# nico-bohlinger/RL-X

Hardware: AMD Instinct MI355X
Metric: env-steps/sec (whole node) PPO 4096 envs at 1/2/4/8 MI355X (higher is better)
Workload: dtype f32

## Files before the change

rl-x_amd/csrc/common.h:

```cpp
#pragma once
#include <hip/hip_runtime.h>
#include <hip/hip_ext.h>
#include <stdint.h>
#include <cstring>
#include <cmath>
#include <string>
#include <vector>
#include <functional>
#include "../../include/rlx_hip.h"

namespace rlx {

void set_error(const std::string& msg);

#define RLX_HIP_TRY(expr)                                                                      \
  do {                                                                                         \
    hipError_t e_ = (expr);                                                                    \
    if (e_ != hipSuccess) {                                                                    \
      ::rlx::set_error(std::string(#expr) + " failed: " + hipGetErrorString(e_) + " (" __FILE__ \
                       ":" + std::to_string(__LINE__) + ")");                                  \
      return RLX_EHIP;                                                                         \
    }                                                                                          \
  } while (0)

// ... 68 lines not shown
  bool pipeline_updates = true;
  bool pf_valid = false;
  uint32_t pf_key_in[2] = {0, 0}, pf_key_out[2] = {0, 0};
  int pf_E = 0, pf_scheme = 0;
  int64_t pf_B = 0;
  hipEvent_t pf_done = nullptr;
  hipEvent_t ev_perm_free = nullptr;
  bool perm_free_recorded = false;
  bool two_streams = true;
  const uint32_t* l1_xmax = nullptr;
  const uint32_t* xmax_slot[2] = {nullptr, nullptr};
  int lf_idle_cus = 0;
  bool dw_recompute = false;
  float* l12_stats = nullptr;
  bool l12_ran = false;
  bool dw_merge = true;
  void* dbg_stamps = nullptr;
  bool fwd2h = true;
  int gather_group_rows = 524288;
  bool gather_records = true;
  bool l12_fused = true;
  int ppo_tail = -1;
  int tail32_waves = 8;
  int ln_row_once = 1;
  int ppo_twin = -1;
  bool fused_recurrent_act = true;
  int num_cus = 256;
  void* defer = nullptr;
  bool prof_on = false;
  int prof_sample = 1;
// ... 376 lines not shown
```

rl-x_amd/csrc/core.hip:

```cpp
#include "common.h"
#include <algorithm>
#include <cstdio>
#include <cstdlib>
#include <utility>

namespace rlx {

static thread_local std::string g_last_error;

void set_error(const std::string& msg) { g_last_error = msg; }

void* scratch(rlx_ctx* ctx, ScratchSlot s, size_t bytes) {
  Scratch& sl = ctx->slots[ctx->bank][s];
  if (sl.bytes >= bytes && sl.ptr) return sl.ptr;
  if (sl.ptr) {
    if (hipDeviceSynchronize() != hipSuccess) { set_error("hipDeviceSynchronize failed in scratch()"); return nullptr; }
    (void)hipFree(sl.ptr);
    sl.ptr = nullptr;
    sl.bytes = 0;
  }
  size_t want = ((bytes > (size_t(1) << 20) ? bytes + bytes / 8 : bytes) + 255) & ~size_t(255);
  void* p = nullptr;
  hipError_t e = hipMalloc(&p, want);
  if (e != hipSuccess) {
// ... 201 lines not shown
  if (std::string(name) == "fwd2h") { ctx->fwd2h = value != 0; return RLX_OK; }
  if (std::string(name) == "l12_fused") { ctx->l12_fused = value != 0; return RLX_OK; }
  if (std::string(name) == "gather_group_rows") { ctx->gather_group_rows = value; return RLX_OK; }
  if (std::string(name) == "gather_records") { ctx->gather_records = value != 0; return RLX_OK; }
  if (std::string(name) == "ppo_tail") { ctx->ppo_tail = value < 0 ? -1 : (value > 2 ? 2 : value); return RLX_OK; }
  if (std::string(name) == "tail32_waves") {
    RLX_REQUIRE(value == 4 || value == 8, RLX_EINVAL, "rlx_dbg_set_option: tail32_waves is 4 or 8");
    ctx->tail32_waves = value;
    return RLX_OK;
  }
  if (std::string(name) == "ln_row_once") {
    RLX_REQUIRE(value == 0 || value == 1, RLX_EINVAL, "rlx_dbg_set_option: ln_row_once is 0 or 1");
    ctx->ln_row_once = value;
    return RLX_OK;
  }
  if (std::string(name) == "bx_force_mi") { ctx->bx_force_mi = value; return RLX_OK; }
  if (std::string(name) == "adam_emit") { ctx->adam_emit = value != 0; return RLX_OK; }
  if (std::string(name) == "bx_debug") { ctx->bx_debug = value; return RLX_OK; }
  if (std::string(name) == "bx_gscale_log2") { ctx->bx_gscale = ldexpf(1.f, value < 0 ? 0 : (value > 40 ? 40 : value)); return RLX_OK; }
  if (std::string(name) == "gemm_bx") { ctx->gemm_bx = value != 0; return RLX_OK; }
  if (std::string(name) == "prof_sample") { ctx->prof_sample = value < 1 ? 1 : value; return RLX_OK; }
  if (std::string(name) == "espo_chunk") { ctx->espo_chunk = value < 1 ? 1 : value; return RLX_OK; }
  if (std::string(name) == "fused_recurrent_act") { ctx->fused_recurrent_act = value != 0; return RLX_OK; }
  RLX_REQUIRE(false, RLX_EINVAL, "rlx_dbg_set_option: unknown option");
}

int rlx_dbg_get_counter(rlx_ctx* ctx, const char* name, int64_t* out) {
  RLX_REQUIRE(ctx && name && out, RLX_EINVAL, "rlx_dbg_get_counter: NULL");
  int bank = 0, slot = 0;
  if (sscanf(name, "scratch_ptr:%d:%d", &bank, &slot) == 2 && bank >= 0 && bank < 3 && slot >= 0 && slot < rlx::SL_COUNT) {
// ... 78 lines not shown
```

rl-x_amd/csrc/l1fused.hip:

```cpp
#include <type_traits>

#include "mlp.h"
#include "gemm_bx.h"

namespace rlx {

#ifndef RLX_LF_PFX
#define RLX_LF_PFX 2
#endif
#ifndef RLX_LF_DWSCALE
#define RLX_LF_DWSCALE 1
#endif
#ifndef RLX_LF_ABL
#define RLX_LF_ABL 0
#endif
#ifndef RLX_LF_STAMPS
#define RLX_LF_STAMPS 0
#endif
constexpr int LF_ROWS = 32;
constexpr int LF_THREADS = 256;
constexpr int LF_XS = 33;
constexpr int LFP_N2 = 256;

typedef float lf_v4 __attribute__((ext_vector_type(4)));
// ... 22 lines not shown
  const float* dZ2;
  const float* W2t;
  const float* W1;
  const float* b1;
  const float* g;
  const float* be;
  float* partials;
  int64_t M;
  int O, H1, N2, act, ln;
  const void* W2x;
  int NTx;
  float gs, gso;
  const void* W1x;
  const uint32_t* xmax;
  unsigned long long* stamps;
};

__device__ __forceinline__ int lf_bx_off(int r, int ks, int N2) { return r * 2 * N2 + ((ks ^ (r & 15)) << 4); }
__device__ __forceinline__ void lf_bx_stage4(char* __restrict__ img, int r, int c4, lf_v4 v, int N2, float sc) {
  uint32_t a0, a1, b0, b1;
  bx_split2(v[0] * sc, v[1] * sc, a0, a1);
  bx_split2(v[2] * sc, v[3] * sc, b0, b1);
  char* d = img + lf_bx_off(r, c4 >> 3, N2) + ((c4 & 4) << 1);
  const int plane = LF_ROWS * 2 * N2;
  *reinterpret_cast<u32x2*>(d) = u32x2{a0, b0};
  *reinterpret_cast<u32x2*>(d + plane) = u32x2{a1, b1};
}

constexpr int LF_XPLANE = LF_ROWS * X_ROWB;
constexpr int LF_XIMG = 2 * X_NP * LF_XPLANE;
__device__ __forceinline__ void lf_x_stage(char* __restrict__ img, int r, int k, float v, float xs) {
  uint32_t p0, p1;
  bx_split2(v * xs, 0.f, p0, p1);
  const int pos = (r & ~12) | ((r & 4) << 1) | ((r & 8) >> 1);
  char* da = img + bx_off(r, k >> 3) + (k & 7) * 2;
  char* dt = img + X_NP * LF_XPLANE + bx_off(k, pos >> 3) + (pos & 7) * 2;
  *reinterpret_cast<uint16_t*>(da) = (uint16_t)p0;
  *reinterpret_cast<uint16_t*>(da + LF_XPLANE) = (uint16_t)p1;
  *reinterpret_cast<uint16_t*>(dt) = (uint16_t)p0;
  *reinterpret_cast<uint16_t*>(dt + LF_XPLANE) = (uint16_t)p1;
}

template <int NT, int NW, int ACT, bool LN, bool BX, bool TWIN = false, bool ROW1 = false>
__global__ __launch_bounds__(64 * NW, NW / 4) void k_dx_l1bwd(L1FusedArgs a, L1FusedArgs a2) {
  if (TWIN && blockIdx.y) a = a2;
  static_assert(!ROW1 || LN, "ROW1 is a form of the LayerNorm statistics");
  constexpr int H1 = 32 * NT * NW;
  constexpr int NTHREADS = 64 * NW;
  extern __shared__ __attribute__((aligned(16))) float smem[];
  const int OP = (a.O + 1) & ~1;
  float* W1s = smem;
  const bool dbuf = a.N2 == LFP_N2;
  const int nbuf = dbuf ? 2 : 1;
  float* As0 = W1s + (BX ? 0 : OP * H1);
  const int a_img = BX ? X_NP * LF_ROWS * a.N2 / 2 : LF_ROWS * (a.N2 + 4);
  float* Xs0 = As0 + nbuf * a_img;
  const int x_img = BX ? LF_XIMG / 4 : LF_ROWS * LF_XS;
  float* red = Xs0 + nbuf * x_img;
  const int t = threadIdx.x, lane = t & 63, w = t >> 6, li = lane & 31, lh = lane >> 5;
  const bool lb0 = (lane & 1) != 0, lb1 = (lane & 2) != 0;
  const int O = a.O, N2 = a.N2;
// ... 21 lines not shown
  }
  const float invH = 1.0f / (float)H1;
  float dw_scale = (RLX_LF_DWSCALE && LN) ? 0.f : a.gs;
  const int AS = N2 + 4;
  const int nq = N2 >> 3;
  constexpr int PF = 4;
  const lf_v4* __restrict__ Wf = reinterpret_cast<const lf_v4*>(a.W2t);
  const u32x4* __restrict__ Wx = reinterpret_cast<const u32x4*>(a.W2x) + (int64_t)(w * NT) * X_NP * 64 + lane;
  const int wx_step = a.NTx * X_NP * 64;
  const u32x4* __restrict__ W1x = reinterpret_cast<const u32x4*>(a.W1x) + (int64_t)(w * NT) * X_NP * 64 + lane;

  const int64_t ntiles = (a.M + LF_ROWS - 1) / LF_ROWS;
  constexpr int SA_N = LF_ROWS * (LFP_N2 / 4) / NTHREADS, SX_N = LF_ROWS * 32 / NTHREADS;
  lf_v4 sa[SA_N];
  float sx[SX_N];
  auto stage_load = [&](int64_t tl) {
    const int64_t rr = tl * LF_ROWS;
#pragma unroll
    for (int c = 0; c < SA_N; ++c) {
      const int i = t + c * NTHREADS, r = i / (LFP_N2 / 4), c4 = (i % (LFP_N2 / 4)) * 4;
      sa[c] = (rr + r < a.M) ? *reinterpret_cast<const lf_v4*>(a.dZ2 + (rr + r) * LFP_N2 + c4) : lf_v4{0.f, 0.f, 0.f, 0.f};
    }
#pragma unroll
    for (int c = 0; c < SX_N; ++c) {
      const int i = t + c * NTHREADS, r = i >> 5, k = i & 31;
      sx[c] = (k < O && rr + r < a.M) ? a.X[(rr + r) * O + k] : 0.f;
    }
  };
  auto stage_store = [&](int b) {
    float* Ad = As0 + b * a_img;
    float* Xd = Xs0 + b * x_img;
#pragma unroll
    for (int c = 0; c < SA_N; ++c) {
      const int i = t + c * NTHREADS, r = i / (LFP_N2 / 4), c4 = (i % (LFP_N2 / 4)) * 4;
      if (BX) lf_bx_stage4(reinterpret_cast<char*>(Ad), r, c4, sa[c], LFP_N2, a.gs);
      else *reinterpret_cast<lf_v4*>(Ad + r * (LFP_N2 + 4) + c4) = sa[c];
    }
#pragma unroll
    for (int c = 0; c < SX_N; ++c) {
      const int i = t + c * NTHREADS;
      if (BX) lf_x_stage(reinterpret_cast<char*>(Xd), i >> 5, i & 31, sx[c], xs);
      else Xd[(i >> 5) * LF_XS + (i & 31)] = sx[c];
    }
  };
  if (dbuf && (int64_t)blockIdx.x < ntiles) {
    stage_load(blockIdx.x);
    stage_store(0);
  }
  int buf = 0;
#if RLX_LF_STAMPS
  int sti = 0;
#define LF_STAMP() if (a.stamps && t == 0 && blockIdx.x == 0 && blockIdx.y == 0 && sti < 18) a.stamps[sti++] = clock64();
#define LF_WALL(I) if (a.stamps && t == 0 && blockIdx.x == 0 && blockIdx.y == 0) a.stamps[I] = wall_clock64();
#define LF_WALL_END() if (sti == 17) { LF_WALL(19) }
#else
#define LF_STAMP()
#define LF_WALL(I)
#define LF_WALL_END()
// ... 30 lines not shown
    if (dbuf) {
      if (has_next) stage_load(tile + gridDim.x);
    } else {
      for (int i = t; i < LF_ROWS * 32; i += NTHREADS) {
        const int r = i >> 5, k = i & 31;
        const float xv = (k < O && r0 + r < a.M) ? a.X[(r0 + r) * O + k] : 0.f;
        if (BX) lf_x_stage(reinterpret_cast<char*>(Xs), r, k, xv, xs);
        else Xs[r * LF_XS + k] = xv;
      }
      for (int i = t; i < LF_ROWS * (N2 >> 2); i += NTHREADS) {
        const int r = i / (N2 >> 2), c4 = (i - r * (N2 >> 2)) * 4;
        const lf_v4 v = (r0 + r < a.M) ? *reinterpret_cast<const lf_v4*>(a.dZ2 + (r0 + r) * N2 + c4) : lf_v4{0.f, 0.f, 0.f, 0.f};
        if (BX) lf_bx_stage4(reinterpret_cast<char*>(As), r, c4, v, N2, a.gs);
        else *reinterpret_cast<lf_v4*>(As + r * AS + c4) = v;
      }
      __syncthreads();
    }
    LF_STAMP()
    const float* a0 = As + li * AS + 4 * lh;
    if (RLX_LF_ABL & 1) {
    } else if (BX) {
      const char* img = reinterpret_cast<const char*>(As);
      const int plane = LF_ROWS * 2 * N2, nb16 = N2 >> 4;
      for (int q = 0; q < nb16; q += PFX) {
#pragma unroll
        for (int u = 0; u < PFX; ++u) {
          u32x4 av[X_NP];
          const char* ab = img + lf_bx_off(li, 2 * (q + u) + lh, N2);
#pragma unroll
          for (int p = 0; p < X_NP; ++p) av[p] = *reinterpret_cast<const u32x4*>(ab + p * plane);
// ... 74 lines not shown
      for (int j = 0; j < NT; ++j)
#pragma unroll
        for (int r = 0; r < 16; ++r) z[j][r] = bias[j];
      const float* x0 = Xs + li * LF_XS + lh;
      const float* w0 = W1s + lh * H1 + w * 32 * NT + li;
      for (int kk = 0; kk < ((RLX_LF_ABL & 8) ? 0 : OP); kk += 2) {
        const float av = x0[kk];
#pragma unroll
        for (int j = 0; j < NT; ++j)
          z[j] = __builtin_amdgcn_mfma_f32_32x32x2f32(av, w0[kk * H1 + 32 * j], z[j], 0, 0, 0);
      }
    }
    LF_STAMP()
    constexpr bool red_on = ln;
    float* redA = red;
    float* redB = red + 2 * NW * 32;
    float* totA = redB + 2 * NW * 32 + w * 64;
    float* totB = redB + 2 * NW * 32 + NW * 64 + w * 64;
    if (red_on) {
#pragma unroll
      for (int g = 0; g < 4; ++g) {
        float sv[4], ssv[4];
#pragma unroll
        for (int e = 0; e < 4; ++e) {
          const int r = 4 * g + e;
          float s = 0.f, ss = 0.f;
#pragma unroll
          for (int j = 0; j < NT; ++j) { s += z[j][r]; ss += z[j][r] * z[j][r]; }
          sv[e] = s;
          ssv[e] = ss;
        }
        const float st = half_sum4(sv[0], sv[1], sv[2], sv[3], lb0, lb1);
        const float sst = half_sum4(ssv[0], ssv[1], ssv[2], ssv[3], lb0, lb1);
        if (li < 4) {
          redA[(0 * NW + w) * 32 + 8 * g + 4 * lh + li] = st;
          redA[(1 * NW + w) * 32 + 8 * g + 4 * lh + li] = sst;
        }
      }
      __syncthreads();
      float rs_row = 0.f;
      {
        float v = 0.f;
#pragma unroll
        for (int q = 0; q < NW; ++q) v += redA[((lane >> 5) * NW + q) * 32 + (lane & 31)];
        totA[lane] = ROW1 ? ln_row_stats(v, lane, invH, rs_row) : v;
      }
      if (BX && RLX_LF_DWSCALE && dw_scale == 0.f) {
        float rs;
        if (ROW1) {
          rs = rs_row;
        } else {
          const float mean = totA[lane & 31] * invH;
          rs = rsqrtf(fmaxf(0.f, totA[32 + (lane & 31)] * invH - mean * mean) + 1e-6f);
        }
        if (r0 + (lane & 31) >= a.M) rs = 0.f;
        rs = fmaxf(rs, dpp_f(rs, 0));
        rs = fmaxf(rs, dpp_f(rs, 1));
        rs = fmaxf(rs, dpp_f(rs, 2));
        rs = fmaxf(rs, dpp_f(rs, 3));
        const unsigned u = (unsigned)__float_as_int(rs);
        const auto r16 = __builtin_amdgcn_permlane16_swap(u, u, false, false);
        rs = fmaxf(__int_as_float((int)r16[0]), __int_as_float((int)r16[1]));
        dw_scale = a.gs * x_pow2_inv(__int_as_float(__builtin_amdgcn_readfirstlane(__float_as_int(rs))));
      }
// ... 128 lines not shown
    {
      const unsigned u0 = (unsigned)__float_as_int(v0), u1 = (unsigned)__float_as_int(v1), u2 = (unsigned)__float_as_int(v2);
      const auto s0 = __builtin_amdgcn_permlane32_swap(u0, u0, false, false);
      const auto s1 = __builtin_amdgcn_permlane32_swap(u1, u1, false, false);
      const auto s2 = __builtin_amdgcn_permlane32_swap(u2, u2, false, false);
      v0 = __int_as_float((int)s0[0]) + __int_as_float((int)s0[1]);
      v1 = __int_as_float((int)s1[0]) + __int_as_float((int)s1[1]);
      v2 = __int_as_float((int)s2[0]) + __int_as_float((int)s2[1]);
    }
    if (lh == 0) {
      out[(int64_t)O * H1 + col] = v0;
      out[(int64_t)(O + 1) * H1 + col] = v1;
      out[(int64_t)(O + 2) * H1 + col] = v2;
    }
  }
}

template <int NT, int NW, int ACT, bool LN, int KS>
__global__ __launch_bounds__(64 * NW, 2) void k_l1fwd_mfma(const float* __restrict__ X, const float* __restrict__ W1,
                                                           const float* __restrict__ b1, const float* __restrict__ g,
                                                           const float* __restrict__ be, float* __restrict__ Hout,
                                                           int64_t M, int O, const int32_t* __restrict__ m_dev,
                                                           int64_t pdelta, float* __restrict__ Hout1) {
  if (blockIdx.y) { W1 += pdelta; b1 += pdelta; g += pdelta; be += pdelta; Hout = Hout1; }
  if (m_dev && (int64_t)*m_dev < M) M = *m_dev;
  constexpr int H1 = 32 * NT * NW;
  constexpr int NTHREADS = 64 * NW;
  extern __shared__ __attribute__((aligned(16))) float smem[];
  const int OP = (O + 1) & ~1;
  float* Xs = smem;
// ... 365 lines not shown
  }
#undef L12_STAMP
#undef L12_WALL
}

bool l12fwd_supported(const rlx_mlp_desc& d) {
  return l1fwd_mfma_supported(d) && d.n_hidden >= 2 && (d.hidden[1] == 256 || d.hidden[1] == 512);
}

int launch_l12fwd(rlx_ctx* ctx, const rlx_mlp_desc& d, const MlpLayout& L, const float* params, const float* x, float* h1, float* h2,
                  const void* w1x, const void* w2x, int64_t M, hipStream_t st, const L12Twin* tw, float* stats) {
  const bool row1 = ctx->ln_row_once != 0;
  const LayerOff &o0 = L.layer[0], &o1 = L.layer[1];
  L12Args a;
  a.X = x; a.W1x = w1x; a.b1 = params + o0.b; a.g = params + o0.g; a.be = params + o0.be; a.W2x = w2x; a.b2 = params + o1.b;
  a.H1 = stats ? nullptr : h1; a.H2 = h2; a.stats = stats; a.xmax = ctx->l1_xmax; a.M = M; a.O = o0.in;
  a.stamps = (unsigned long long*)ctx->dbg_stamps;
  L12Args a2 = a;
  if (tw) {
    a2.W1x = tw->w1x; a2.b1 = tw->params + o0.b; a2.g = tw->params + o0.g; a2.be = tw->params + o0.be; a2.W2x = tw->w2x;
    a2.b2 = tw->params + o1.b; a2.H1 = stats ? nullptr : tw->h1; a2.H2 = tw->h2; a2.stats = tw->stats;
  }
  const int N2 = o1.out;
  const double nets = tw ? 2.0 : 1.0;
  ProfScope prof(ctx, PK_L12FWD, nets * 2.0 * (double)M * L12_H1 * (N2 + o0.in), st,
                 nets * 4.0 * ((double)M * (o0.in + (stats ? 2 : L12_H1) + N2) + (double)L12_H1 * (N2 + o0.in)), M, N2, L12_H1, 1);
  const int64_t nt = (M + LF_ROWS - 1) / LF_ROWS;
  const int per = tw ? ctx->num_cus : 2 * ctx->num_cus;
  const int grid = (int)(nt < per ? nt : per);
  const size_t lds = (size_t)X_NP * LF_ROWS * L12_AROW + 2 * X_NP * LF_XPLANE + (2 * 8 * 32 + 8 * 64) * sizeof(float);
#define RLX_L12_ATTR(...)                                                                                          \
  RLX_HIP_TRY(hipFuncSetAttribute(reinterpret_cast<const void*>(k_l12fwd<__VA_ARGS__>), hipFuncAttributeMaxDynamicSharedMemorySize, 160 * 1024));
#define RLX_L12_LAUNCH_ROW(NT2V, ROWV)                                                                             \
  {                                                                                                                \
    static AttrOnce attr_set;                                                                                        \
    if (!attr_set.done()) {                                                                                               \
      RLX_L12_ATTR(RLX_ACT_ELU, NT2V, false, false, ROWV)                                                          \
      RLX_L12_ATTR(RLX_ACT_ELU, NT2V, true, false, ROWV)                                                           \
      RLX_L12_ATTR(RLX_ACT_ELU, NT2V, false, true, ROWV)                                                           \
      attr_set.mark();                                                                                               \
    }                                                                                                              \
// ... 92 lines not shown
                       H1, N2);
    RLX_LAUNCH_CHECK();
  }
  L1FusedArgs a;
  a.X = x; a.dZ2 = dZ2; a.W2t = W2t; a.W1 = params + o0.W; a.b1 = params + o0.b;
  a.g = o0.g >= 0 ? params + o0.g : nullptr;
  a.be = o0.be >= 0 ? params + o0.be : nullptr;
  a.partials = slabs; a.M = M; a.O = O; a.H1 = H1; a.N2 = N2; a.act = d.act; a.ln = d.ln_first ? 1 : 0;
  a.W2x = w2x;
  a.W1x = w1x;
  a.NTx = 4 * div_up(H1, G_BN);
  a.gs = ctx->bx_gscale;
  a.gso = X_WINV / a.gs;
  a.xmax = ctx->l1_xmax;
  a.stamps = RLX_LF_STAMPS ? (unsigned long long*)ctx->dbg_stamps : nullptr;
  L1FusedArgs a2 = a;
  if (tw) {
    a2.dZ2 = tw->dZ2; a2.W1 = tw->params + o0.W; a2.b1 = tw->params + o0.b;
    a2.g = o0.g >= 0 ? tw->params + o0.g : nullptr;
    a2.be = o0.be >= 0 ? tw->params + o0.be : nullptr;
    a2.partials = tw->arena; a2.W2x = tw->w2x; a2.W1x = tw->w1x;
  }
  const int OP = (O + 1) & ~1;
  const size_t a_img = bxk ? (size_t)X_NP * LF_ROWS * N2 / 2 : (size_t)LF_ROWS * (N2 + 4);
  const size_t lds = bxk ? ((N2 == LFP_N2 ? 2 : 1) * (a_img + LF_XIMG / 4) + 2048) * sizeof(float)
                         : ((size_t)OP * H1 + (N2 == LFP_N2 ? 2 : 1) * (a_img + LF_ROWS * LF_XS) + 2048) * sizeof(float);
  RLX_REQUIRE(lds <= 160 * 1024, RLX_EUNSUP, "l1fused: tile image exceeds the LDS");
  {
    const double ntw = tw ? 2.0 : 1.0;
    ProfScope prof(ctx, PK_DX_L1BWD, ntw * 2.0 * (double)M * H1 * (N2 + O), st,
                   ntw * 4.0 * ((double)M * N2 + (double)H1 * N2 + (double)M * O + 2.0 * O * H1), M, H1, N2, bxk ? 1 : 0);
#define RLX_LF_ATTR(KERNEL)                                                                                    \
  {                                                                                                            \
    static AttrOnce attr_set;                                                                                    \
    if (!attr_set.done()) {                                                                                           \
      RLX_HIP_TRY(hipFuncSetAttribute(reinterpret_cast<const void*>(KERNEL), hipFuncAttributeMaxDynamicSharedMemorySize, \
                                      160 * 1024));                                                            \
      attr_set.mark();                                                                                           \
    }                                                                                                          \
  }
#define RLX_LF_LAUNCH(NTV, NWV, ACTV, LNV)                                                                      \
  {                                                                                                            \
    RLX_LF_ATTR((k_dx_l1bwd<NTV, NWV, ACTV, LNV, false>))                                                      \
    RLX_LF_ATTR((k_dx_l1bwd<NTV, NWV, ACTV, LNV, true>))                                                       \
    RLX_LF_ATTR((k_dx_l1bwd<NTV, NWV, ACTV, LNV, true, true>))                                                 \
    if (tw) { RLX_PLAUNCH((k_dx_l1bwd<NTV, NWV, ACTV, LNV, true, true>), dim3(grid, 2), dim3(64 * NWV), lds, st, a, a2); } \
    else if (bxk) { RLX_PLAUNCH((k_dx_l1bwd<NTV, NWV, ACTV, LNV, true>), dim3(grid), dim3(64 * NWV), lds, st, a, a2); } \
    else { RLX_PLAUNCH((k_dx_l1bwd<NTV, NWV, ACTV, LNV, false>), dim3(grid), dim3(64 * NWV), lds, st, a, a2); }    \
  }
#define RLX_LF_LAUNCH_ROW1(NTV, NWV, ACTV)                                                                      \
  {                                                                                                            \
    RLX_LF_ATTR((k_dx_l1bwd<NTV, NWV, ACTV, true, true, false, true>))                                         \
    RLX_LF_ATTR((k_dx_l1bwd<NTV, NWV, ACTV, true, true, true, true>))                                          \
    if (tw) { RLX_PLAUNCH((k_dx_l1bwd<NTV, NWV, ACTV, true, true, true, true>), dim3(grid, 2), dim3(64 * NWV), lds, st, a, a2); } \
    else { RLX_PLAUNCH((k_dx_l1bwd<NTV, NWV, ACTV, true, true, false, true>), dim3(grid), dim3(64 * NWV), lds, st, a, a2); } \
  }
    if (H1 == 512 && d.act == RLX_ACT_ELU && d.ln_first && bxk && ctx->ln_row_once) RLX_LF_LAUNCH_ROW1(2, 8, RLX_ACT_ELU)
    else
    if (H1 == 512 && d.act == RLX_ACT_ELU && d.ln_first) RLX_LF_LAUNCH(2, 8, RLX_ACT_ELU, true)
    else if (H1 == 256 && d.act == RLX_ACT_TANH && !d.ln_first) RLX_LF_LAUNCH(2, 4, RLX_ACT_TANH, false)
    else if (H1 == 256 && d.act == RLX_ACT_RELU && !d.ln_first) RLX_LF_LAUNCH(2, 4, RLX_ACT_RELU, false)
    else RLX_REQUIRE(false, RLX_EUNSUP, "l1fused: unsupported (hidden[0], act, ln) combination");
#undef RLX_LF_LAUNCH_ROW1
#undef RLX_LF_LAUNCH
#undef RLX_LF_ATTR
  }
  RLX_LAUNCH_CHECK();
  const int64_t PS = (int64_t)(O + 3) * H1;
  tab->seg[tab->n++] = ReduceSeg{slabs, grads + o0.W, (int64_t)O * H1, PS, grid, 0, 1.f, 0.f, 1};
  tab->seg[tab->n++] = ReduceSeg{slabs + (int64_t)O * H1, grads + o0.b, (int64_t)H1, PS, grid, 0, 1.f, 0.f, 1};
  if (d.ln_first) {
    tab->seg[tab->n++] = ReduceSeg{slabs + (int64_t)(O + 1) * H1, grads + o0.g, (int64_t)H1, PS, grid, 0, 1.f, 0.f, 1};
    tab->seg[tab->n++] = ReduceSeg{slabs + (int64_t)(O + 2) * H1, grads + o0.be, (int64_t)H1, PS, grid, 0, 1.f, 0.f, 1};
  }
  if (tw) {
    ReduceTable* t2 = tw->tab;
    float* s2 = tw->arena;
// ... 12 lines not shown
```

rl-x_amd/csrc/mlp.hip:

```cpp
#include "mlp.h"
#include "ln_kernels.h"

namespace rlx {

constexpr int L1_R_FWD = 4, L1_R_BWD = 2;
constexpr int L1_MAXJ = 8;
constexpr int L1_THREADS = 512;

__device__ __forceinline__ float readlane_f(float v, int lane) {
  return __int_as_float(__builtin_amdgcn_readlane(__float_as_int(v), lane));
}

struct L1Args {
  const float* X;
  float* H;
  int64_t M;
  int O, Hd, NJ;
};

template <bool BWD, int ACT, bool LN, int L1R>
__device__ __forceinline__ void l1_rows(const L1Args& a, const float* __restrict__ Ws, const float* __restrict__ bs,
                                        const float* __restrict__ gs, const float* __restrict__ bes,
                                        float (&dg)[L1_MAXJ], float (&dbe)[L1_MAXJ], int lane, int64_t wave_g,
                                        int64_t nwaves) {
// ... 951 lines not shown
  RLX_LAUNCH_CHECK();
  return RLX_OK;
}

int mlp_trunk_fwd(rlx_ctx* ctx, const rlx_mlp_desc& d, const MlpLayout& L, const float* params, const float* x,
                  float* const* acts, int64_t M, hipStream_t st, int ldx, bool gemm_l0, const int32_t* m_dev, int n_layers) {
  int rc;
  const int nl = (n_layers >= 1 && n_layers <= d.n_hidden) ? n_layers : d.n_hidden;
  int l_next = 1;
  if (ctx->l12_fused && d.in_dim <= 32 && !gemm_l0 && !m_dev && nl >= 2 && M >= 4096 && (ldx <= 0 || ldx == d.in_dim) &&
      l12fwd_supported(d)) {
    const LayerOff &o0 = L.layer[0], &o1 = L.layer[1];
    const void* w1x = bx_lookup(ctx, params + o0.W, 0, o0.in, o0.out);
    const void* w2x = w1x ? bx_lookup(ctx, params + o1.W, 0, o1.in, o1.out) : nullptr;
    if (w1x && w2x) {
      rc = launch_l12fwd(ctx, d, L, params, x, acts[0], acts[1], w1x, w2x, M, st, nullptr, ctx->l12_stats);
      if (rc) return rc;
      l_next = 2;
      ctx->l12_ran = ctx->l12_stats != nullptr;
    }
  }
  if (l_next == 2) {
  } else if (d.in_dim <= 32 && !gemm_l0) {
    RLX_REQUIRE(ldx <= 0 || ldx == d.in_dim, RLX_EUNSUP, "mlp: padded input rows need in_dim > 32");
    rc = launch_l1_fwd(d, L, params, x, acts[0], M, ctx->num_cus, st, ctx->l1fwd_mfma, m_dev, ctx);
  } else {
    const LayerOff& o = L.layer[0];
    const int ld = ldx > 0 ? ldx : d.in_dim;
    RLX_REQUIRE(ld % 4 == 0 && ld >= d.in_dim, RLX_EUNSUP, "mlp: wide inputs need a row stride that is a multiple of 4");
    if (d.ln_first) {
      RLX_REQUIRE(acts[3] != nullptr && d.n_hidden >= 2, RLX_EUNSUP, "mlp: wide LayerNorm layer without its pre-activation buffer");
// ... 596 lines not shown
```

rl-x_amd/csrc/ppo.hip:

```cpp
#include "ppo_internal.h"
#include "gemm_bx.h"
#include "dist.h"

namespace rlx {

constexpr float LOG_2PI = 1.8378770664093453f;
constexpr float HALF_LOG_2PIE = 1.4189385332046727f;
constexpr int HEAD_ROWS = 64;

__global__ __launch_bounds__(256) void k_gather(const float* __restrict__ states, const float* __restrict__ actions,
                                                const float* __restrict__ logp, const float* __restrict__ returns,
                                                const float* __restrict__ adv, const int32_t* __restrict__ idx,
                                                float* __restrict__ mb_x, float* __restrict__ mb_a,
                                                float* __restrict__ aux, const int32_t* __restrict__ valid_rows,
                                                int64_t mb, int O, int A, const float* __restrict__ cstates,
                                                float* __restrict__ mb_xc, int Oc) {
  const int64_t nv = valid_rows ? (int64_t)*valid_rows : mb;
  const int64_t nx = mb * O, na = mb * A, nxc = cstates ? mb * Oc : 0;
  const int64_t total = nx + na + mb + nxc;
  for (int64_t e = (int64_t)blockIdx.x * 256 + threadIdx.x; e < total; e += (int64_t)gridDim.x * 256) {
    if (e >= nx + na + mb) {
      const int64_t f = e - nx - na - mb;
      const int64_t r = f / Oc;
      const int d = (int)(f - r * Oc);
// ... 1385 lines not shown
    if (K == 64) RLX_HL_FAST(16)
    else if (K == 128) RLX_HL_FAST(32)
    else RLX_HL_FAST(64)
#undef RLX_HL_FAST
    RLX_LAUNCH_CHECK();
    return RLX_OK;
  }
  const size_t lds = ((size_t)HEAD_ROWS * (K + 1) + (size_t)K * A + 2 * (size_t)HEAD_ROWS * A + 2 * A) * sizeof(float);
  RLX_REQUIRE(lds <= 160 * 1024, RLX_EUNSUP, "ppo head: last hidden layer too wide for the LDS-staged head kernel");
  hipLaunchKernelGGL(k_head_loss<POLICY>, dim3(nb), dim3(256), lds, st, H, W, b, logstd, s.mb_a, s.aux, s.stats, s.head_part,
                     metrics, mb, K, A, PS, inv_mb, hp.clip_range, hp.entropy_coef, hp.critic_coef, act, s.valid_rows);
  RLX_LAUNCH_CHECK();
  return RLX_OK;
}

template <bool POLICY>
static int net_fwd_bwd(rlx_ctx* ctx, const rlx_mlp_desc& d, const float* params, float* grads, float* metrics,
                       const MbScratch& s, int64_t mb, int mb_global, const rlx_ppo_hparams& hp, float* sumsq,
                       int* n_sumsq, hipStream_t st, hipEvent_t ev_after_fwd = nullptr) {
  const MlpLayout L = make_layout(d);
  const bool kept = ctx->bx_keep[ctx->bank] && ctx->bx_n[ctx->bank] > 0 && d.n_hidden >= 2 &&
                    ctx->bx_img[ctx->bank][0].W == params + L.layer[1].W;
  int rc = (mb >= 4096 && !kept) ? bx_prepare_mlp(ctx, d, L, params, true, st) : RLX_OK;
  if (rc) return rc;
  struct BxScope { rlx_ctx* c; ~BxScope() { if (!c->bx_keep[c->bank]) bx_release(c); } } bx_scope{ctx};
  const float* x_in = (!POLICY && s.mb_xc) ? s.mb_xc : s.mb_x;
  const int K = L.head.in, A = L.head.out;
  const int PS = K * A + 2 * A + 8;
  int nb = div_up(mb, HEAD_ROWS);
  const float inv_mb = 1.0f / (float)mb_global;
  const bool discrete = POLICY && hp.discrete_actions != 0;
  const void *w3f = nullptr, *w3t = nullptr;
  float* dz2 = nullptr;
  if (tail_shape_ok(ctx, d, mb, hp)) {
    const LayerOff& o3 = L.layer[2];
    w3f = bx_lookup(ctx, params + o3.W, 0, o3.in, o3.out);
    w3t = bx_lookup(ctx, params + o3.W, 1, o3.out, o3.in);
    if (w3f && w3t) dz2 = (float*)scratch(ctx, SL_DACT_0, (size_t)mb * o3.in * sizeof(float));
  }
  const bool tail = dz2 != nullptr;
  if (tail) nb = (int)(mb / tail_rows(ctx, L.layer[2].in, d.act, mb));
  XmaxScope xscope(ctx, ctx->xmax_slot[(!POLICY && s.mb_xc) ? 1 : 0]);
  struct L12Scope { rlx_ctx* c; ~L12Scope() { c->l12_stats = nullptr; c->l12_ran = false; } } l12scope{ctx};
  ctx->l12_ran = false;
  ctx->l12_stats = nullptr;
  if (ctx->dw_recompute && tail && ctx->l12_fused && l12fwd_supported(d) && dw_merge_ok(ctx, d, L, mb) && d.hidden[0] == 512 &&
      d.act == RLX_ACT_ELU && grads) {
    ctx->l12_stats = (float*)scratch(ctx, SL_LN_P, (size_t)2 * mb * sizeof(float));
    if (!ctx->l12_stats) return RLX_ENOMEM;
  }
  rc = mlp_trunk_fwd(ctx, d, L, params, x_in, s.acts, mb, st, 0, false, nullptr, tail ? d.n_hidden - 1 : -1);
  if (rc) return rc;
  if (ev_after_fwd) RLX_HIP_TRY(hipEventRecord(ev_after_fwd, st));
  if (tail) {
    const LayerOff& o3 = L.layer[2];
    const TailNet tn{s.acts[1], (const u32x4*)w3f, (const u32x4*)w3t, params + o3.b, params + L.head.W, params + L.head.b,
                     POLICY ? params + L.logstd : nullptr, s.acts[2], dz2, s.head_part, A, PS};
    rc = launch_tail(ctx, POLICY ? &tn : nullptr, POLICY ? nullptr : &tn, s, metrics, mb, o3.in, mb_global, hp, d.act, st);
  } else {
    rc = launch_head_loss<POLICY>(s.acts[d.n_hidden - 1], params + L.head.W, params + L.head.b,
                                  (POLICY && !discrete) ? params + L.logstd : nullptr, s, metrics, mb, K, A, PS, inv_mb, hp,
                                  d.act, st, ctx);
  }
  if (rc) return rc;
// ... 86 lines not shown
  *ok = true;
  return RLX_OK;
}

static int twin_fwd_bwd(rlx_ctx* ctx, const rlx_mlp_desc& pd, const MlpLayout& LP, const float* pparams, float* pg,
                        const rlx_mlp_desc& cd, const MlpLayout& LC, const float* cparams, float* cg, const TwinImages& im,
                        float* met, const MbScratch& sp, const MbScratch& sc, int64_t mb, int mb_global,
                        const rlx_ppo_hparams& hp, float* sq, int* npb, int* ncb, hipStream_t st) {
  const int nh = pd.n_hidden, last = nh - 1;
  Twin t;
  XmaxScope xscope(ctx, ctx->xmax_slot[0]);
  int rc;
  int l_first = 1;
  float* stats2[2] = {nullptr, nullptr};
  const bool l12 = ctx->l12_fused && l12fwd_supported(pd) && im.w1x[0] && im.w1x[1];
  if (l12 && ctx->dw_recompute && ctx->dw_merge && nh == 3 && tail_shape_ok(ctx, pd, mb, hp) && pd.hidden[0] == 512 &&
      pd.act == RLX_ACT_ELU) {
    const int b0 = ctx->bank;
    for (int q = 0; q < 2; ++q) {
      ctx->bank = q;
      stats2[q] = (float*)scratch(ctx, SL_LN_P, (size_t)2 * mb * sizeof(float));
    }
    ctx->bank = b0;
    if (!stats2[0] || !stats2[1]) return RLX_ENOMEM;
  }
  if (l12) {
    L12Twin tw{cparams, sc.acts[0], sc.acts[1], im.w1x[1], im.f[1][1]};
    tw.stats = stats2[1];
    rc = launch_l12fwd(ctx, pd, LP, pparams, sp.mb_x, sp.acts[0], sp.acts[1], im.w1x[0], im.f[1][0], mb, st, &tw, stats2[0]);
    l_first = 2;
  } else {
    rc = launch_l1fwd_mfma(pd, LP, pparams, sp.mb_x, sp.acts[0], mb, ctx->num_cus, st, nullptr, ctx, cparams, sc.acts[0]);
  }
  if (rc) return rc;
  float* dz2[2] = {nullptr, nullptr};
  const float* dzb[4][2];
  for (int l = 0; l < 4; ++l) { dzb[l][0] = sp.acts[l]; dzb[l][1] = sc.acts[l]; }
  if (tail_shape_ok(ctx, pd, mb, hp)) {
    const int bank0_ = ctx->bank;
    for (int q = 0; q < 2; ++q) {
      ctx->bank = q;
      dz2[q] = (float*)scratch(ctx, SL_DACT_0, (size_t)mb * LP.layer[2].in * sizeof(float));
    }
    ctx->bank = bank0_;
// ... 61 lines not shown
      pB[l][q] = cur; cur += (size_t)S[l] * o.out;
    }
    lf[q] = cur;
  }
  float* gr[2] = {pg, cg};
  const MlpLayout* LL[2] = {&LP, &LC};
  ReduceTable tab[2];
  tab[0].n = tab[1].n = 0;
  for (int l = last; l >= 1; --l) {
    const LayerOff& o = LP.layer[l];
    if (dw_merge) {
      if (l == 1) {
        const LayerOff& o3 = LP.layer[2];
        BxDwJob j2{sp.acts[0], dzb[1][0], pW[1][0], pB[1][0], o.in, o.in, o.out, Mc[1], S[1], div_up(o.in, G_BM), div_up(o.out, G_BN)};
        BxDwRecompute rcd;
        if (stats2[0]) {
          const LayerOff& o0 = LP.layer[0];
          rcd.X = sp.mb_x; rcd.W1x = im.w1x[0]; rcd.b1 = pparams + o0.b; rcd.g = pparams + o0.g; rcd.be = pparams + o0.be;
          rcd.stats = stats2[0]; rcd.xmax = ctx->l1_xmax; rcd.W1x1 = im.w1x[1]; rcd.stats1 = stats2[1];
          rcd.pdelta1 = (int64_t)(cparams - pparams); rcd.O = o0.in; rcd.NT1 = o0.out / 32;
          j2.rc = &rcd;
        }
        const BxDwJob j3{sp.acts[1], dzb[2][0], pW[2][0], pB[2][0], o3.in, o3.in, o3.out, Mc[2], S[2], div_up(o3.in, G_BM), div_up(o3.out, G_BN)};
        Twin t2, t3;
        t2.p[0] = sc.acts[0]; t2.p[1] = dzb[1][1]; t2.p[2] = pW[1][1]; t2.p[3] = pB[1][1];
        t3.p[0] = sc.acts[1]; t3.p[1] = dzb[2][1]; t3.p[2] = pW[2][1]; t3.p[3] = pB[2][1];
        rc = bx_launch_dw2(ctx, j2, j3, mb, st, &t2, &t3);
        if (rc) return rc;
      }
    } else {
      t.p[0] = sc.acts[l - 1]; t.p[1] = dzb[l][1]; t.p[2] = pW[l][1]; t.p[3] = pB[l][1];
// ... 910 lines not shown
```

Before: 7.951 million.

## Hand over layer-1 LayerNorm row statistics from fused forward to dx backward kernel

The fused layer-1/2 forward kernel now writes per-row LayerNorm statistics even when it also stores H1, and the layer-1 backward kernel gains a variant that loads these statistics instead of recomputing row sums and sums of squares with a cross-wave LDS reduction and barrier. This removes a reduction pass and a __syncthreads from each backward tile, and uses a smaller LDS reduction area. In exchange it adds global writes and reads of two floats per row, more context plumbing and scope resets, and a new kernel variant.

New measurement: 8.104 million, median of 6. +1.9%, better.

```diff
diff --git a/rl-x_amd/csrc/common.h b/rl-x_amd/csrc/common.h
--- a/rl-x_amd/csrc/common.h
+++ b/rl-x_amd/csrc/common.h
@@ -106,6 +106,9 @@
   bool dw_recompute = false;
   float* l12_stats = nullptr;
   bool l12_ran = false;
+  int l1_stats_handover = 1;
+  float* l1_hand_req = nullptr;
+  const float* l1_hand[2] = {nullptr, nullptr};
   bool dw_merge = true;
   void* dbg_stamps = nullptr;
   bool fwd2h = true;
diff --git a/rl-x_amd/csrc/core.hip b/rl-x_amd/csrc/core.hip
--- a/rl-x_amd/csrc/core.hip
+++ b/rl-x_amd/csrc/core.hip
@@ -239,6 +239,11 @@
     ctx->ln_row_once = value;
     return RLX_OK;
   }
+  if (std::string(name) == "l1_stats_handover") {
+    RLX_REQUIRE(value == 0 || value == 1, RLX_EINVAL, "rlx_dbg_set_option: l1_stats_handover is 0 or 1");
+    ctx->l1_stats_handover = value;
+    return RLX_OK;
+  }
   if (std::string(name) == "bx_force_mi") { ctx->bx_force_mi = value; return RLX_OK; }
   if (std::string(name) == "adam_emit") { ctx->adam_emit = value != 0; return RLX_OK; }
   if (std::string(name) == "bx_debug") { ctx->bx_debug = value; return RLX_OK; }
diff --git a/rl-x_amd/csrc/l1fused.hip b/rl-x_amd/csrc/l1fused.hip
--- a/rl-x_amd/csrc/l1fused.hip
+++ b/rl-x_amd/csrc/l1fused.hip
@@ -60,7 +60,10 @@
   const void* W1x;
   const uint32_t* xmax;
   unsigned long long* stamps;
+  const float* stats;
 };
+constexpr int LF_RED = 2048;
+constexpr int LF_RED_HAND = 2 * 64 + 2 * 8 * 32 + 8 * 64;
 
 __device__ __forceinline__ int lf_bx_off(int r, int ks, int N2) { return r * 2 * N2 + ((ks ^ (r & 15)) << 4); }
 __device__ __forceinline__ void lf_bx_stage4(char* __restrict__ img, int r, int c4, lf_v4 v, int N2, float sc) {
@@ -87,10 +90,11 @@
   *reinterpret_cast<uint16_t*>(dt + LF_XPLANE) = (uint16_t)p1;
 }
 
-template <int NT, int NW, int ACT, bool LN, bool BX, bool TWIN = false, bool ROW1 = false>
-__global__ __launch_bounds__(64 * NW, NW / 4) void k_dx_l1bwd(L1FusedArgs a, L1FusedArgs a2) {
+template <int NT, int NW, int ACT, bool LN, bool BX, bool TWIN, bool ROW1, bool HAND>
+__device__ __forceinline__ void lf_dx_l1bwd(L1FusedArgs a, const L1FusedArgs& a2) {
   if (TWIN && blockIdx.y) a = a2;
   static_assert(!ROW1 || LN, "ROW1 is a form of the LayerNorm statistics");
+  static_assert(!HAND || (ROW1 && BX), "HAND takes the statistics of k_l12fwd<ROW1>: the split-operand LayerNorm form only");
   constexpr int H1 = 32 * NT * NW;
   constexpr int NTHREADS = 64 * NW;
   extern __shared__ __attribute__((aligned(16))) float smem[];
@@ -142,34 +146,49 @@
   constexpr int SA_N = LF_ROWS * (LFP_N2 / 4) / NTHREADS, SX_N = LF_ROWS * 32 / NTHREADS;
   lf_v4 sa[SA_N];
   float sx[SX_N];
+  float sh = 0.f;
+  auto hand_load = [&](int64_t rr, int tt) -> float {
+    const float* sb = a.stats + rr;
+    const uint32_t off = (uint32_t)(tt >> 5) * (uint32_t)a.M + (uint32_t)(tt & 31);
+    return rr + (tt & 31) < a.M ? sb[off] : (tt < 32 ? 0.f : 1.f);
+  };
+  auto t_opaque = [&]() -> int {
+    int tt = t;
+    if (HAND) asm volatile("" : "+v"(tt));
+    return tt;
+  };
   auto stage_load = [&](int64_t tl) {
     const int64_t rr = tl * LF_ROWS;
+    const int ts = t_opaque();
+    if (HAND && ts < 64) sh = hand_load(rr, ts);
 #pragma unroll
     for (int c = 0; c < SA_N; ++c) {
-      const int i = t + c * NTHREADS, r = i / (LFP_N2 / 4), c4 = (i % (LFP_N2 / 4)) * 4;
+      const int i = ts + c * NTHREADS, r = i / (LFP_N2 / 4), c4 = (i % (LFP_N2 / 4)) * 4;
       sa[c] = (rr + r < a.M) ? *reinterpret_cast<const lf_v4*>(a.dZ2 + (rr + r) * LFP_N2 + c4) : lf_v4{0.f, 0.f, 0.f, 0.f};
     }
 #pragma unroll
     for (int c = 0; c < SX_N; ++c) {
-      const int i = t + c * NTHREADS, r = i >> 5, k = i & 31;
+      const int i = ts + c * NTHREADS, r = i >> 5, k = i & 31;
       sx[c] = (k < O && rr + r < a.M) ? a.X[(rr + r) * O + k] : 0.f;
     }
   };
   auto stage_store = [&](int b) {
     float* Ad = As0 + b * a_img;
     float* Xd = Xs0 + b * x_img;
+    const int ts = t_opaque();
 #pragma unroll
     for (int c = 0; c < SA_N; ++c) {
-      const int i = t + c * NTHREADS, r = i / (LFP_N2 / 4), c4 = (i % (LFP_N2 / 4)) * 4;
+      const int i = ts + c * NTHREADS, r = i / (LFP_N2 / 4), c4 = (i % (LFP_N2 / 4)) * 4;
       if (BX) lf_bx_stage4(reinterpret_cast<char*>(Ad), r, c4, sa[c], LFP_N2, a.gs);
       else *reinterpret_cast<lf_v4*>(Ad + r * (LFP_N2 + 4) + c4) = sa[c];
     }
 #pragma unroll
     for (int c = 0; c < SX_N; ++c) {
-      const int i = t + c * NTHREADS;
+      const int i = ts + c * NTHREADS;
       if (BX) lf_x_stage(reinterpret_cast<char*>(Xd), i >> 5, i & 31, sx[c], xs);
       else Xd[(i >> 5) * LF_XS + (i & 31)] = sx[c];
     }
+    if (HAND && ts < 64) red[b * 64 + ts] = sh;
   };
   if (dbuf && (int64_t)blockIdx.x < ntiles) {
     stage_load(blockIdx.x);
@@ -230,6 +249,7 @@
         if (BX) lf_bx_stage4(reinterpret_cast<char*>(As), r, c4, v, N2, a.gs);
         else *reinterpret_cast<lf_v4*>(As + r * AS + c4) = v;
       }
+      if (HAND && t < 64) red[t] = hand_load(r0, t);
       __syncthreads();
     }
     LF_STAMP()
@@ -334,40 +354,44 @@
     LF_STAMP()
     constexpr bool red_on = ln;
     float* redA = red;
-    float* redB = red + 2 * NW * 32;
-    float* totA = redB + 2 * NW * 32 + w * 64;
-    float* totB = redB + 2 * NW * 32 + NW * 64 + w * 64;
+    float* redB = red + (HAND ? 2 * 64 : 2 * NW * 32);
+    float* totA = HAND ? red + buf * 64 : redB + 2 * NW * 32 + w * 64;
+    float* totB = redB + 2 * NW * 32 + (HAND ? 0 : NW * 64) + w * 64;
     if (red_on) {
-#pragma unroll
-      for (int g = 0; g < 4; ++g) {
-        float sv[4], ssv[4];
-#pragma unroll
-        for (int e = 0; e < 4; ++e) {
-          const int r = 4 * g + e;
-          float s = 0.f, ss = 0.f;
-#pragma unroll
-          for (int j = 0; j < NT; ++j) { s += z[j][r]; ss += z[j][r] * z[j][r]; }
-          sv[e] = s;
-          ssv[e] = ss;
-        }
-        const float st = half_sum4(sv[0], sv[1], sv[2], sv[3], lb0, lb1);
-        const float sst = half_sum4(ssv[0], ssv[1], ssv[2], ssv[3], lb0, lb1);
-        if (li < 4) {
-          redA[(0 * NW + w) * 32 + 8 * g + 4 * lh + li] = st;
-          redA[(1 * NW + w) * 32 + 8 * g + 4 * lh + li] = sst;
-        }
-      }
-      __syncthreads();
       float rs_row = 0.f;
-      {
-        float v = 0.f;
-#pragma unroll
-        for (int q = 0; q < NW; ++q) v += redA[((lane >> 5) * NW + q) * 32 + (lane & 31)];
-        totA[lane] = ROW1 ? ln_row_stats(v, lane, invH, rs_row) : v;
+      if (!HAND) {
+#pragma unroll
+        for (int g = 0; g < 4; ++g) {
+          float sv[4], ssv[4];
+#pragma unroll
+          for (int e = 0; e < 4; ++e) {
+            const int r = 4 * g + e;
+            float s = 0.f, ss = 0.f;
+#pragma unroll
+            for (int j = 0; j < NT; ++j) { s += z[j][r]; ss += z[j][r] * z[j][r]; }
+            sv[e] = s;
+            ssv[e] = ss;
+          }
+          const float st = half_sum4(sv[0], sv[1], sv[2], sv[3], lb0, lb1);
+          const float sst = half_sum4(ssv[0], ssv[1], ssv[2], ssv[3], lb0, lb1);
+          if (li < 4) {
+            redA[(0 * NW + w) * 32 + 8 * g + 4 * lh + li] = st;
+            redA[(1 * NW + w) * 32 + 8 * g + 4 * lh + li] = sst;
+          }
+        }
+        __syncthreads();
+        {
+          float v = 0.f;
+#pragma unroll
+          for (int q = 0; q < NW; ++q) v += redA[((lane >> 5) * NW + q) * 32 + (lane & 31)];
+          totA[lane] = ROW1 ? ln_row_stats(v, lane, invH, rs_row) : v;
+        }
       }
       if (BX && RLX_LF_DWSCALE && dw_scale == 0.f) {
         float rs;
-        if (ROW1) {
+        if (HAND) {
+          rs = totA[32 + (lane & 31)];
+        } else if (ROW1) {
           rs = rs_row;
         } else {
           const float mean = totA[lane & 31] * invH;
@@ -526,6 +550,16 @@
       out[(int64_t)(O + 2) * H1 + col] = v2;
     }
   }
+}
+
+template <int NT, int NW, int ACT, bool LN, bool BX, bool TWIN = false, bool ROW1 = false>
+__global__ __launch_bounds__(64 * NW, NW / 4) void k_dx_l1bwd(L1FusedArgs a, L1FusedArgs a2) {
+  lf_dx_l1bwd<NT, NW, ACT, LN, BX, TWIN, ROW1, false>(a, a2);
+}
+
+template <int NT, int NW, int ACT, bool TWIN>
+__global__ __launch_bounds__(64 * NW, NW / 4) void k_dx_l1bwd_stats(L1FusedArgs a, L1FusedArgs a2) {
+  lf_dx_l1bwd<NT, NW, ACT, true, true, TWIN, true, true>(a, a2);
 }
 
 template <int NT, int NW, int ACT, bool LN, int KS>
@@ -921,17 +955,19 @@
   const LayerOff &o0 = L.layer[0], &o1 = L.layer[1];
   L12Args a;
   a.X = x; a.W1x = w1x; a.b1 = params + o0.b; a.g = params + o0.g; a.be = params + o0.be; a.W2x = w2x; a.b2 = params + o1.b;
-  a.H1 = stats ? nullptr : h1; a.H2 = h2; a.stats = stats; a.xmax = ctx->l1_xmax; a.M = M; a.O = o0.in;
+  a.H1 = h1; a.H2 = h2; a.stats = stats; a.xmax = ctx->l1_xmax; a.M = M; a.O = o0.in;
   a.stamps = (unsigned long long*)ctx->dbg_stamps;
   L12Args a2 = a;
   if (tw) {
     a2.W1x = tw->w1x; a2.b1 = tw->params + o0.b; a2.g = tw->params + o0.g; a2.be = tw->params + o0.be; a2.W2x = tw->w2x;
-    a2.b2 = tw->params + o1.b; a2.H1 = stats ? nullptr : tw->h1; a2.H2 = tw->h2; a2.stats = tw->stats;
-  }
+    a2.b2 = tw->params + o1.b; a2.H1 = tw->h1; a2.H2 = tw->h2; a2.stats = tw->stats;
+  }
+  ctx->l1_hand[0] = row1 ? a.stats : nullptr;
+  ctx->l1_hand[1] = (row1 && tw) ? a2.stats : nullptr;
   const int N2 = o1.out;
   const double nets = tw ? 2.0 : 1.0;
   ProfScope prof(ctx, PK_L12FWD, nets * 2.0 * (double)M * L12_H1 * (N2 + o0.in), st,
-                 nets * 4.0 * ((double)M * (o0.in + (stats ? 2 : L12_H1) + N2) + (double)L12_H1 * (N2 + o0.in)), M, N2, L12_H1, 1);
+                 nets * 4.0 * ((double)M * (o0.in + (stats ? 2 : 0) + (h1 ? L12_H1 : 0) + N2) + (double)L12_H1 * (N2 + o0.in)), M, N2, L12_H1, 1);
   const int64_t nt = (M + LF_ROWS - 1) / LF_ROWS;
   const int per = tw ? ctx->num_cus : 2 * ctx->num_cus;
   const int grid = (int)(nt < per ? nt : per);
@@ -1054,22 +1090,26 @@
   a.gso = X_WINV / a.gs;
   a.xmax = ctx->l1_xmax;
   a.stamps = RLX_LF_STAMPS ? (unsigned long long*)ctx->dbg_stamps : nullptr;
+  const bool row1k = H1 == 512 && d.act == RLX_ACT_ELU && d.ln_first && bxk && ctx->ln_row_once;
+  const bool hand = row1k && ctx->l1_stats_handover && ctx->l1_hand[0] && (!tw || ctx->l1_hand[1]) && M < ((int64_t)1 << 30);
+  a.stats = hand ? ctx->l1_hand[0] : nullptr;
   L1FusedArgs a2 = a;
   if (tw) {
     a2.dZ2 = tw->dZ2; a2.W1 = tw->params + o0.W; a2.b1 = tw->params + o0.b;
     a2.g = o0.g >= 0 ? tw->params + o0.g : nullptr;
     a2.be = o0.be >= 0 ? tw->params + o0.be : nullptr;
     a2.partials = tw->arena; a2.W2x = tw->w2x; a2.W1x = tw->w1x;
+    a2.stats = hand ? ctx->l1_hand[1] : nullptr;
   }
   const int OP = (O + 1) & ~1;
   const size_t a_img = bxk ? (size_t)X_NP * LF_ROWS * N2 / 2 : (size_t)LF_ROWS * (N2 + 4);
-  const size_t lds = bxk ? ((N2 == LFP_N2 ? 2 : 1) * (a_img + LF_XIMG / 4) + 2048) * sizeof(float)
-                         : ((size_t)OP * H1 + (N2 == LFP_N2 ? 2 : 1) * (a_img + LF_ROWS * LF_XS) + 2048) * sizeof(float);
+  const size_t lds = bxk ? ((N2 == LFP_N2 ? 2 : 1) * (a_img + LF_XIMG / 4) + (hand ? LF_RED_HAND : LF_RED)) * sizeof(float)
+                         : ((size_t)OP * H1 + (N2 == LFP_N2 ? 2 : 1) * (a_img + LF_ROWS * LF_XS) + LF_RED) * sizeof(float);
   RLX_REQUIRE(lds <= 160 * 1024, RLX_EUNSUP, "l1fused: tile image exceeds the LDS");
   {
     const double ntw = tw ? 2.0 : 1.0;
     ProfScope prof(ctx, PK_DX_L1BWD, ntw * 2.0 * (double)M * H1 * (N2 + O), st,
-                   ntw * 4.0 * ((double)M * N2 + (double)H1 * N2 + (double)M * O + 2.0 * O * H1), M, H1, N2, bxk ? 1 : 0);
+                   ntw * 4.0 * ((double)M * (N2 + (hand ? 2 : 0)) + (double)H1 * N2 + (double)M * O + 2.0 * O * H1), M, H1, N2, bxk ? 1 : 0);
 #define RLX_LF_ATTR(KERNEL)                                                                                    \
   {                                                                                                            \
     static AttrOnce attr_set;                                                                                    \
@@ -1095,12 +1135,21 @@
     if (tw) { RLX_PLAUNCH((k_dx_l1bwd<NTV, NWV, ACTV, true, true, true, true>), dim3(grid, 2), dim3(64 * NWV), lds, st, a, a2); } \
     else { RLX_PLAUNCH((k_dx_l1bwd<NTV, NWV, ACTV, true, true, false, true>), dim3(grid), dim3(64 * NWV), lds, st, a, a2); } \
   }
-    if (H1 == 512 && d.act == RLX_ACT_ELU && d.ln_first && bxk && ctx->ln_row_once) RLX_LF_LAUNCH_ROW1(2, 8, RLX_ACT_ELU)
+#define RLX_LF_LAUNCH_HAND(NTV, NWV, ACTV)                                                                      \
+  {                                                                                                            \
+    RLX_LF_ATTR((k_dx_l1bwd_stats<NTV, NWV, ACTV, false>))                                                     \
+    RLX_LF_ATTR((k_dx_l1bwd_stats<NTV, NWV, ACTV, true>))                                                      \
+    if (tw) { RLX_PLAUNCH((k_dx_l1bwd_stats<NTV, NWV, ACTV, true>), dim3(grid, 2), dim3(64 * NWV), lds, st, a, a2); } \
+    else { RLX_PLAUNCH((k_dx_l1bwd_stats<NTV, NWV, ACTV, false>), dim3(grid), dim3(64 * NWV), lds, st, a, a2); } \
+  }
+    if (hand) RLX_LF_LAUNCH_HAND(2, 8, RLX_ACT_ELU)
+    else if (row1k) RLX_LF_LAUNCH_ROW1(2, 8, RLX_ACT_ELU)
     else
     if (H1 == 512 && d.act == RLX_ACT_ELU && d.ln_first) RLX_LF_LAUNCH(2, 8, RLX_ACT_ELU, true)
     else if (H1 == 256 && d.act == RLX_ACT_TANH && !d.ln_first) RLX_LF_LAUNCH(2, 4, RLX_ACT_TANH, false)
     else if (H1 == 256 && d.act == RLX_ACT_RELU && !d.ln_first) RLX_LF_LAUNCH(2, 4, RLX_ACT_RELU, false)
     else RLX_REQUIRE(false, RLX_EUNSUP, "l1fused: unsupported (hidden[0], act, ln) combination");
+#undef RLX_LF_LAUNCH_HAND
 #undef RLX_LF_LAUNCH_ROW1
 #undef RLX_LF_LAUNCH
 #undef RLX_LF_ATTR
diff --git a/rl-x_amd/csrc/mlp.hip b/rl-x_amd/csrc/mlp.hip
--- a/rl-x_amd/csrc/mlp.hip
+++ b/rl-x_amd/csrc/mlp.hip
@@ -989,7 +989,8 @@
     const void* w1x = bx_lookup(ctx, params + o0.W, 0, o0.in, o0.out);
     const void* w2x = w1x ? bx_lookup(ctx, params + o1.W, 0, o1.in, o1.out) : nullptr;
     if (w1x && w2x) {
-      rc = launch_l12fwd(ctx, d, L, params, x, acts[0], acts[1], w1x, w2x, M, st, nullptr, ctx->l12_stats);
+      rc = launch_l12fwd(ctx, d, L, params, x, ctx->l12_stats ? nullptr : acts[0], acts[1], w1x, w2x, M, st, nullptr,
+                         ctx->l12_stats ? ctx->l12_stats : ctx->l1_hand_req);
       if (rc) return rc;
       l_next = 2;
       ctx->l12_ran = ctx->l12_stats != nullptr;
diff --git a/rl-x_amd/csrc/ppo.hip b/rl-x_amd/csrc/ppo.hip
--- a/rl-x_amd/csrc/ppo.hip
+++ b/rl-x_amd/csrc/ppo.hip
@@ -1423,6 +1423,11 @@
   return RLX_OK;
 }
 
+static bool l1_handover_wanted(const rlx_ctx* ctx, const rlx_mlp_desc& d, int64_t mb) {
+  return ctx->l1_stats_handover && ctx->ln_row_once && ctx->gemm_bx && ctx->l12_fused && !ctx->disable_l1fused && mb >= 4096 &&
+         l12fwd_supported(d) && l1fused_supported(d);
+}
+
 template <bool POLICY>
 static int net_fwd_bwd(rlx_ctx* ctx, const rlx_mlp_desc& d, const float* params, float* grads, float* metrics,
                        const MbScratch& s, int64_t mb, int mb_global, const rlx_ppo_hparams& hp, float* sumsq,
@@ -1450,13 +1455,21 @@
   const bool tail = dz2 != nullptr;
   if (tail) nb = (int)(mb / tail_rows(ctx, L.layer[2].in, d.act, mb));
   XmaxScope xscope(ctx, ctx->xmax_slot[(!POLICY && s.mb_xc) ? 1 : 0]);
-  struct L12Scope { rlx_ctx* c; ~L12Scope() { c->l12_stats = nullptr; c->l12_ran = false; } } l12scope{ctx};
+  struct L12Scope {
+    rlx_ctx* c;
+    ~L12Scope() { c->l12_stats = nullptr; c->l12_ran = false; c->l1_hand_req = nullptr; c->l1_hand[0] = c->l1_hand[1] = nullptr; }
+  } l12scope{ctx};
   ctx->l12_ran = false;
   ctx->l12_stats = nullptr;
+  ctx->l1_hand_req = nullptr;
+  ctx->l1_hand[0] = ctx->l1_hand[1] = nullptr;
   if (ctx->dw_recompute && tail && ctx->l12_fused && l12fwd_supported(d) && dw_merge_ok(ctx, d, L, mb) && d.hidden[0] == 512 &&
       d.act == RLX_ACT_ELU && grads) {
     ctx->l12_stats = (float*)scratch(ctx, SL_LN_P, (size_t)2 * mb * sizeof(float));
     if (!ctx->l12_stats) return RLX_ENOMEM;
+  } else if (l1_handover_wanted(ctx, d, mb) && grads) {
+    ctx->l1_hand_req = (float*)scratch(ctx, SL_LN_P, (size_t)2 * mb * sizeof(float));
+    if (!ctx->l1_hand_req) return RLX_ENOMEM;
   }
   rc = mlp_trunk_fwd(ctx, d, L, params, x_in, s.acts, mb, st, 0, false, nullptr, tail ? d.n_hidden - 1 : -1);
   if (rc) return rc;
@@ -1573,8 +1586,11 @@
   int l_first = 1;
   float* stats2[2] = {nullptr, nullptr};
   const bool l12 = ctx->l12_fused && l12fwd_supported(pd) && im.w1x[0] && im.w1x[1];
-  if (l12 && ctx->dw_recompute && ctx->dw_merge && nh == 3 && tail_shape_ok(ctx, pd, mb, hp) && pd.hidden[0] == 512 &&
-      pd.act == RLX_ACT_ELU) {
+  struct HandScope { rlx_ctx* c; ~HandScope() { c->l1_hand[0] = c->l1_hand[1] = nullptr; } } hand_scope{ctx};
+  ctx->l1_hand[0] = ctx->l1_hand[1] = nullptr;
+  const bool no_h1 = l12 && ctx->dw_recompute && ctx->dw_merge && nh == 3 && tail_shape_ok(ctx, pd, mb, hp) && pd.hidden[0] == 512 &&
+                     pd.act == RLX_ACT_ELU;
+  if (no_h1 || (l12 && l1_handover_wanted(ctx, pd, mb))) {
     const int b0 = ctx->bank;
     for (int q = 0; q < 2; ++q) {
       ctx->bank = q;
@@ -1584,9 +1600,9 @@
     if (!stats2[0] || !stats2[1]) return RLX_ENOMEM;
   }
   if (l12) {
-    L12Twin tw{cparams, sc.acts[0], sc.acts[1], im.w1x[1], im.f[1][1]};
+    L12Twin tw{cparams, no_h1 ? nullptr : sc.acts[0], sc.acts[1], im.w1x[1], im.f[1][1]};
     tw.stats = stats2[1];
-    rc = launch_l12fwd(ctx, pd, LP, pparams, sp.mb_x, sp.acts[0], sp.acts[1], im.w1x[0], im.f[1][0], mb, st, &tw, stats2[0]);
+    rc = launch_l12fwd(ctx, pd, LP, pparams, sp.mb_x, no_h1 ? nullptr : sp.acts[0], sp.acts[1], im.w1x[0], im.f[1][0], mb, st, &tw, stats2[0]);
     l_first = 2;
   } else {
     rc = launch_l1fwd_mfma(pd, LP, pparams, sp.mb_x, sp.acts[0], mb, ctx->num_cus, st, nullptr, ctx, cparams, sc.acts[0]);
@@ -1678,7 +1694,7 @@
         const LayerOff& o3 = LP.layer[2];
         BxDwJob j2{sp.acts[0], dzb[1][0], pW[1][0], pB[1][0], o.in, o.in, o.out, Mc[1], S[1], div_up(o.in, G_BM), div_up(o.out, G_BN)};
         BxDwRecompute rcd;
-        if (stats2[0]) {
+        if (no_h1) {
           const LayerOff& o0 = LP.layer[0];
           rcd.X = sp.mb_x; rcd.W1x = im.w1x[0]; rcd.b1 = pparams + o0.b; rcd.g = pparams + o0.g; rcd.be = pparams + o0.be;
           rcd.stats = stats2[0]; rcd.xmax = ctx->l1_xmax; rcd.W1x1 = im.w1x[1]; rcd.stats1 = stats2[1];
```
